# Indra-jith/failure-aware-vision

Measured on AMD Instinct MI355X. Metric: frames/sec, ResNet-50 MC-Dropout T=30 224x224 batch=256, higher is better.
Workload: dtype bf16; 1 GPU; BASELINE configs[2]: ResNet-50 v1.5 + MC-Dropout T=30 (all_blocks, p=0.10), 224x224x3 fp32 frames with Gaussian noise severity 3, batch 256 per GPU, synthetic frames and seeded synthetic weights; frames_per_gpu=256, global_batch=256, mc_samples=30, dropout_policy=all_blocks, inputs=resident in HBM before the timed region (H2D excluded), parallelism=batch sharded, 1 process per GPU, all-gather of (label, confidence)

## Files before the change

### failure_aware_vision_amd/csrc/fav.hip

```cpp
#include <hip/hip_runtime.h>

#include <algorithm>
#include <atomic>
#include <climits>
#include <cmath>
#include <cstdio>
#include <cstdlib>
#include <cstring>
#include <string>
#include <vector>

#include "../../include/fav.h"
#include "fav_kernels.hpp"
#include "fav_corrupt_c.hpp"
#include "fav_plan.hpp"
#include "fav_route.hpp"
#include "fav_views.hpp"
#include "fav_ood.hpp"
#include "fav_knn.hpp"

using namespace fav_plan;
using namespace fav_route;

namespace {
// ... 197 lines not shown
    igemm<128, 128, 64, 2, 0, 0>(), igemm<128, 128, 64, 2, 0, 1>(), igemm<128, 128, 64, 2, 0, 0, 0, true>(), igemm<128, 128, 64, 2, 0, 1, 0, true>(),
    igemm<128, 128, 64, 2, 1, 0>(), igemm<128, 128, 64, 2, 1, 1>(), igemm<128, 128, 64, 2, 1, 0, 0, true>(), igemm<128, 128, 64, 2, 1, 1, 0, true>(),
    igemm<256, 256, 64, 2, 0, 1, 1>(), igemm<256, 256, 64, 2, 0, 1, 1, true>(),
    igemm<256, 256, 64, 2, 0, 0>(), igemm<256, 256, 64, 2, 0, 1>(), igemm<256, 256, 64, 2, 0, 0, 0, true>(), igemm<256, 256, 64, 2, 0, 1, 0, true>(),
    igemm<256, 256, 64, 2, 1, 0>(), igemm<256, 256, 64, 2, 1, 1>(), igemm<256, 256, 64, 2, 1, 0, 0, true>(), igemm<256, 256, 64, 2, 1, 1, 0, true>(),
};
const KernelEntry<HaloKernel> kHaloKernels[] = {
    halo<64, 64, 256, 3, 1, 4, 0>(), halo<64, 64, 256, 3, 1, 4, 1>(), halo<128, 128, 256, 2, 2, 2, 0>(), halo<128, 128, 256, 2, 2, 2, 1>(),
    halo<64, 64, 128, 2, 1, 3, 0>(), halo<64, 64, 128, 2, 1, 3, 1>(), halo<128, 128, 128, 2, 1, 2, 0>(), halo<128, 128, 128, 2, 1, 2, 1>(),
};
const KernelEntry<TailKernel> kTailKernels[] = {
    tail<64, 0, true, 3, 4, true>(), tail<64, 0, true, 3, 4, false>(), tail<64, 64, true, 3, 4, true>(), tail<64, 64, true, 3, 4, false>(),
    tail<64, 128, true, 3, 4, true>(), tail<64, 128, true, 3, 4, false>(),
    tail<64, 0, false, 3, 4, true>(), tail<64, 0, false, 3, 4, false>(), tail<64, 64, false, 3, 4, true>(), tail<64, 64, false, 3, 4, false>(),
    tail<64, 128, false, 3, 4, true>(), tail<64, 128, false, 3, 4, false>(),
    tail<128, 0, true, 2, 8, true>(), tail<128, 0, true, 2, 8, false>(), tail<128, 128, true, 2, 8, true>(), tail<128, 128, true, 2, 8, false>(),
    tail<128, 0, false, 2, 8, true>(), tail<128, 0, false, 2, 8, false>(), tail<128, 128, false, 2, 8, true>(), tail<128, 128, false, 2, 8, false>(),
    tail<512, 0, false, 2, 8, true>(), tail<256, 0, true, 2, 8, true>(), tail<256, 0, false, 2, 4, true>(), tail<256, 0, false, 2, 4, false>(),
    tail<256, 256, false, 2, 8, true, 16>(), tail<256, 256, false, 2, 8, false, 16>(),
    tail<64, 64, true, 3, 4, true, 32, true>(), tail<64, 64, true, 3, 4, false, 32, true>(),
    {ROUTE_PROJ, {256, 512, 4}, bottleneck_tail_kernel<256, 0, false, 2, 4, true, 32, 512, false, false>},
    {ROUTE_PROJ, {512, 1024, 8}, bottleneck_tail_kernel<512, 0, false, 2, 8, true, 32, 1024, false, false>},
};
const KernelEntry<AttnKernel> kAttnKernels[] = {attn<0, 13, true>(), attn<0, 13>(), attn<0, 16>(), attn<1, 13>(), attn<1, 16>()};

template <class Fn, size_t N>
Fn find_kernel(const KernelEntry<Fn> (&table)[N], const Route& r, bool* lds_ok) {
    *lds_ok = true;
    for (const KernelEntry<Fn>& e : table) {
        if (e.kind != r.kind || memcmp(e.a, r.a, sizeof r.a) != 0) continue;
        if (r.lds > 0 && !e.lds_set.test_current()) {
            *lds_ok = hipFuncSetAttribute((const void*)e.fn, hipFuncAttributeMaxDynamicSharedMemorySize, 160 * 1024) == hipSuccess;
            if (*lds_ok) e.lds_set.set_current();
        }
        return e.fn;
    }
    return nullptr;
}

TailParams tail_params(const Route& r) {
    TailParams p;
    memset(&p, 0, sizeof p);
    p.H = r.Ho; p.W = r.Wo; p.HW = r.Ho * r.Wo; p.M = r.M;
    p.in_W = p.W; p.in_HW = p.HW; p.in_stride = 1;
    const TailGeom& g = r.geom;
    p.rega_bytes = g.rega_bytes;
    p.bias_b_off = g.bias_b_off; p.bias_ca_off = g.bias_ca_off; p.wa_off0 = g.wa_off0; p.wa_off1 = g.wa_off1; p.zero_off = g.zero_off;
    p.div_hw = fastdiv_make((uint32_t)p.HW);
    p.div_w = fastdiv_make((uint32_t)p.W);
    p.rs_T = r.rs_T; p.rs_tps = r.rs_tps;
    return p;
}

const char* launch_proj(fav_handle* h, const fav_conv_desc& d, const Route& r, const Group& G, hipStream_t s) {
    TailParams p = tail_params(r);
    p.t1 = (const uint16_t*)d.x; p.wc = (const uint16_t*)d.w; p.bias_c = d.bias; p.y = (uint16_t*)d.y;
    p.in_W = d.W; p.in_HW = d.H * d.W; p.in_stride = d.stride;
    p.drop = make_drop(nullptr);
    p.g_t1 = G.x; p.g_wc = G.w; p.g_bc = G.b; p.g_y = G.y;
    bool lds_ok;
    const TailKernel kern = find_kernel(kTailKernels, r, &lds_ok);
    if (!kern || !lds_ok) return kern ? "conv: cannot reserve LDS for the projection kernel" : "conv: no kernel for this route";
    const double flops = 2.0 * (double)r.M * d.Cin * d.Cout * G.n;
    const double bytes = 2.0 * ((double)r.M * (d.Cin + d.Cout) + (double)d.Cin * d.Cout) * G.n;
    Prof pr(h, s, FAV_K_CONV, flops, bytes);
    g_route = r;
    hipLaunchKernelGGL(kern, dim3(r.grid, r.groups), dim3(r.block), r.lds, s, p, 0);
    return nullptr;
}

const char* launch_conv(fav_handle* h, const fav_conv_desc& d, int cout_pad, int ldy, bool vit, const Group& G, hipStream_t s) {
    const Route r = route_conv(d, cout_pad, ldy, vit, G.n);
    if (r.refusal) return r.refusal;
    if (r.kind == ROUTE_PROJ) return launch_proj(h, d, r, G, s);
    ConvParams p;
    p.x = (const uint16_t*)d.x; p.w = (const uint16_t*)d.w; p.bias = d.bias; p.res = (const uint16_t*)d.res; p.y = d.y;
    p.H = d.H; p.W = d.W; p.Cin = d.Cin;
    p.Ho = r.Ho; p.Wo = r.Wo; p.HWo = r.Ho * r.Wo;
    p.Cout = d.Cout; p.ldy = ldy;
    p.kw = d.kw; p.stride = d.stride; p.pad = d.pad;
    p.M = r.M; p.K = r.K; p.nk = r.nk;
    p.relu = d.relu; p.out_f32 = d.out_f32;
    p.tiles_m = r.tiles_m; p.tiles_n = r.tiles_n; p.stage_mid = r.stage_mid;
    p.drop = make_drop(&d.drop);
    p.div_hwo = fastdiv_make((uint32_t)p.HWo);
    p.div_w = fastdiv_make((uint32_t)p.Wo);
    p.dbg = nullptr;
    p.g_x = G.x; p.g_w = G.w; p.g_bias = G.b; p.g_res = G.res; p.g_y = G.y;
    const bool halo = r.kind == ROUTE_CONV_HALO;
    bool lds_ok;
    const HaloKernel kern_halo = halo ? find_kernel(kHaloKernels, r, &lds_ok) : nullptr;
    const ConvKernel kern = halo ? nullptr : find_kernel(kConvKernels, r, &lds_ok);
    if (!kern_halo && !kern) return "conv: no kernel for this route";
    if (!lds_ok) return "conv: cannot reserve LDS for the staged 3x3 kernel";
    const double flops = 2.0 * (double)r.M * d.Cout * r.K * G.n;
    const double bytes = 2.0 * ((double)d.n_frames * d.H * d.W * d.Cin + (double)r.M * d.Cout * (d.res ? 2 : 1) * (d.out_f32 ? 2 : 1)
                                + (double)d.Cout * r.K) * G.n;
    const long long tiles = (long long)r.tiles_m * r.tiles_n;
    const bool dbg_on = FAV_KNOB("FAV_CONV_DBG", 0) != 0;
    if (dbg_on && !h) { (void)hipMalloc((void**)&p.dbg, (size_t)tiles * 32); (void)hipMemset(p.dbg, 0, (size_t)tiles * 32); }
    auto dbg_report = [&](long long nblocks, int bm, int bn, int bk) {
        if (!p.dbg) return;
        (void)hipStreamSynchronize(s);
        std::vector<unsigned long long> t((size_t)nblocks * 4);
        (void)hipMemcpy(t.data(), p.dbg, t.size() * 8, hipMemcpyDeviceToHost);
        (void)hipFree(p.dbg);
        unsigned long long lo = ~0ull, hi = 0;
        double ph[3] = {0, 0, 0};
        for (long long i = 0; i < nblocks; ++i) {
            lo = std::min(lo, t[i * 4]); hi = std::max(hi, t[i * 4 + 3]);
            for (int j = 0; j < 3; ++j) ph[j] += (double)(t[i * 4 + j + 1] - t[i * 4 + j]);
        }
        const double span = (double)(hi - lo), life = ph[0] + ph[1] + ph[2];
        fprintf(stderr, "[conv dbg] blocks %lld BMxBNxBK %dx%dx%d span %.1f us; per block: prologue %.2f us, k-loop %.2f us, epilogue %.2f us; "
                        "resident blocks/CU %.2f\n", nblocks, bm, bn, bk, span / 100.0, ph[0] / nblocks / 100.0, ph[1] / nblocks / 100.0,
                ph[2] / nblocks / 100.0, life / span / 256.0);
    };
    Prof pr(h, s, FAV_K_CONV, flops, bytes);
    g_route = r;
    if (halo) hipLaunchKernelGGL(kern_halo, dim3(r.grid, r.groups), dim3(r.block), r.lds, s, p, r.patch_bytes);
    else hipLaunchKernelGGL(kern, dim3(r.grid, r.groups), dim3(r.block), 0, s, p);
    dbg_report(r.grid, halo ? r.a[2] : r.a[0], r.a[1], halo ? 64 : r.a[2]);
    return nullptr;
}

const char* launch_tail(fav_handle* h, const fav_tail_desc& d, const Group& G, hipStream_t s) {
    const Route r = route_tail(d, G.n);
    if (r.refusal) return r.refusal;
    TailParams p = tail_params(r);
    p.t1 = (const uint16_t*)d.x; p.wb = (const uint16_t*)d.wb; p.bias_b = d.bias_b;
    p.wc = (const uint16_t*)d.wc; p.bias_c = d.bias_c; p.res = (const uint16_t*)d.res; p.y = (uint16_t*)d.y;
    p.wa = (const uint16_t*)d.wa; p.bias_a = d.bias_a; p.t1n = (uint16_t*)d.t1n;
    p.drop = make_drop(&d.drop);
    p.g_t1 = G.x; p.g_res = G.res; p.g_y = G.y; p.g_t1n = G.y2;
    p.g_wb = G.wb; p.g_bb = G.bb; p.g_wc = G.w; p.g_bc = G.b; p.g_wa = G.wa; p.g_ba = G.ba;
    p.site_e = d.entry_site;
    bool lds_ok;
    const TailKernel kern = find_kernel(kTailKernels, r, &lds_ok);
    if (!kern) return "bottleneck tail: unsupported shape";
    if (!lds_ok) return "bottleneck tail: cannot reserve LDS";
    const int cmid = d.Cmid, cout = 4 * cmid, nred = r.a[1], bm = r.geom.rp * r.geom.nw;
    const bool has3x3 = r.a[2] != 0;
    const long long M = r.M, nblocks = r.grid;
    const double flops = 2.0 * (double)M * ((has3x3 ? 9.0 * cmid * cmid : 0.0) + (double)cmid * cout + (double)cout * nred) * G.n;
    const double res_rows = d.res_entry ? (double)std::min<long long>(d.n_frames, p.drop.n_img) * p.HW : (double)M;
    const double bytes = 2.0 * ((double)M * (cmid + 1.0 * cout + nred) + res_rows * cout + (has3x3 ? 9.0 * cmid * cmid : 0.0) + (double)cmid * cout + (double)cout * nred) * G.n;
    Prof pr(h, s, FAV_K_CONV, flops, bytes);
    const bool dbg_on = FAV_KNOB("FAV_CONV_DBG", 0) != 0;
    if (dbg_on && !h) { (void)hipMalloc((void**)&p.dbg, (size_t)nblocks * 128); (void)hipMemset(p.dbg, 0, (size_t)nblocks * 128); }
    auto dbg_report = [&]() {
        if (!p.dbg) return;
        (void)hipStreamSynchronize(s);
        std::vector<unsigned long long> t((size_t)nblocks * 16);
        (void)hipMemcpy(t.data(), p.dbg, t.size() * 8, hipMemcpyDeviceToHost);
        (void)hipFree(p.dbg);
        if (const char* dump = fav_knob_str("FAV_CONV_DBG_DUMP")) {
            if (FILE* f = fopen(dump, "ab")) { const long long hdr[2] = {nblocks, cmid * 1000 + nred}; fwrite(hdr, 8, 2, f); fwrite(t.data(), 8, t.size(), f); fclose(f); }
        }
        unsigned long long lo = ~0ull, hi = 0;
        double ph[5] = {0, 0, 0, 0, 0};
        double cy[5] = {0, 0, 0, 0, 0};
        double cz[3] = {0, 0, 0};
        for (long long i = 0; i < nblocks; ++i) {
            lo = std::min(lo, t[i * 16]); hi = std::max(hi, t[i * 16 + 5]);
            unsigned long long prev = t[i * 16];
            for (int j = 0; j < 5; ++j) { const unsigned long long c = t[i * 16 + j + 1] ? t[i * 16 + j + 1] : prev; ph[j] += (double)(c - prev); prev = c; }
// ... 1907 lines not shown
```

### failure_aware_vision_amd/csrc/fav_kernels.hpp

```cpp
#pragma once
#include <hip/hip_runtime.h>
#include <float.h>
#include <stdint.h>

#ifdef FAV_EXPERIMENTS
#define FAV_DBG(P) ((P).dbg)
#else
#define FAV_DBG(P) ((unsigned long long*)nullptr)
#endif

namespace fav {

typedef __attribute__((__vector_size__(8 * sizeof(__bf16)))) __bf16 bf16x8_t;
typedef __attribute__((__vector_size__(4 * sizeof(float)))) float f32x4_t;

__device__ __forceinline__ float bf16_bits_to_f32(uint32_t b) { return __uint_as_float(b << 16); }

__device__ __forceinline__ uint32_t f32_to_bf16_bits(float f) {
    uint32_t u = __float_as_uint(f);
    return (u + 0x7FFFu + ((u >> 16) & 1u)) >> 16;
}
typedef __bf16 bf16x2_t __attribute__((ext_vector_type(2)));
typedef float f32x2_t __attribute__((ext_vector_type(2)));
typedef uint32_t u32x4_t __attribute__((ext_vector_type(4)));
// ... 328 lines not shown
            f32x4_t acc[4];
#pragma unroll
            for (int a = 0; a < 4; ++a) acc[a] = f32x4_t{0.f, 0.f, 0.f, 0.f};
#pragma unroll
            for (int s = 0; s < 6; ++s) {
                union { uint4 u; bf16x8_t v; } ub;
                ub.u = make_uint4(0, 0, 0, 0);
                if (s < 5) {
                    const StemFrag f = *(const StemFrag*)(win + 64 * s);
                    ub.u = s < 4 ? make_uint4(f.x, f.y, f.z, f.w) : make_uint4(f.x & km0, f.y & km1, f.z & km23, f.w & km23);
                }
#pragma unroll
                for (int a = 0; a < 4; ++a) {
                    union { uint4 u; bf16x8_t v; } ua;
                    ua.u = wf[a][s];
                    acc[a] = __builtin_amdgcn_mfma_f32_16x16x32_bf16(ua.v, ub.v, acc[a], 0, 0, 0);
                }
            }
            char* crow = (char*)conv_s + q * 128 + ((fq & 1) << 3);
#pragma unroll
            for (int a = 0; a < 4; ++a) {
                const float4 bq = *(const float4*)(bias_s + 16 * a + 4 * fq);
                const float v0 = __fadd_rn(acc[a][0], bq.x), v1 = __fadd_rn(acc[a][1], bq.y);
                const float v2 = __fadd_rn(acc[a][2], bq.z), v3 = __fadd_rn(acc[a][3], bq.w);
                *(uint2*)(crow + (((2 * a + (fq >> 1)) ^ (q & 7)) << 4)) = make_uint2(relu_bf16x2(pack_bf16x2(v0, v1)), relu_bf16x2(pack_bf16x2(v2, v3)));
            }
        }
        __syncthreads();

#pragma unroll
        for (int it = 0; it < 2; ++it) {
            const int item = tid + 256 * it;
            const int u = item & 7, pp = item >> 3;
            const int ppy = pp >> 3, ppx = pp & 7;
            const int gpy = py0 + ppy, gpx = px0 + ppx;
            if (gpy < p.Hp && gpx < p.Wp) {
                const int qm = (2 * ppy + 1) * CT + 2 * ppx + 1;
                u16x2_t best[4] = {{0, 0}, {0, 0}, {0, 0}, {0, 0}};
#pragma unroll
                for (int r = 0; r < 3; ++r) {
                    const bool rok = (unsigned)(2 * gpy - 1 + r) < (unsigned)p.Hc;
#pragma unroll
                    for (int s = 0; s < 3; ++s) {
                        const bool ok = rok && (unsigned)(2 * gpx - 1 + s) < (unsigned)p.Wc;
                        const int q = ok ? qm + (r - 1) * CT + (s - 1) : qm;
                        const uint4 v = *(const uint4*)((const char*)conv_s + q * 128 + ((u ^ (q & 7)) << 4));
                        best[0] = __builtin_elementwise_max(best[0], __builtin_bit_cast(u16x2_t, v.x));
                        best[1] = __builtin_elementwise_max(best[1], __builtin_bit_cast(u16x2_t, v.y));
                        best[2] = __builtin_elementwise_max(best[2], __builtin_bit_cast(u16x2_t, v.z));
                        best[3] = __builtin_elementwise_max(best[3], __builtin_bit_cast(u16x2_t, v.w));
                    }
                }
                *(uint4*)(p.out + (((img * p.Hp + gpy) * p.Wp + gpx) << 6) + 8 * u) =
                    make_uint4(__builtin_bit_cast(uint32_t, best[0]), __builtin_bit_cast(uint32_t, best[1]),
                               __builtin_bit_cast(uint32_t, best[2]), __builtin_bit_cast(uint32_t, best[3]));
            }
        }
    }
#undef FAV_STEM_REQUEST
}

__device__ __forceinline__ void lds_dma16(__amdgpu_buffer_rsrc_t srd, uint32_t voff, uint32_t soff, uint32_t lds_addr) {
    asm volatile("s_mov_b32 m0, %0\n\ts_nop 0\n\tbuffer_load_dwordx4 %1, %2, %3 offen lds"
                 :
                 : "s"(lds_addr), "v"(voff), "s"(srd), "s"(soff)
                 : "memory", "m0");
}

struct ConvParams {
    const uint16_t* x;
    const uint16_t* w;
    const float* bias;
    const uint16_t* res;
    void* y;
    int H, W, Cin, Ho, Wo, HWo;
    int Cout;
    int ldy;
    int kw, stride, pad;
    int M;
    int K, nk;
    int relu, out_f32;
    int tiles_m, tiles_n;
    int stage_mid;
    DropParams drop;
    FastDiv div_hwo;
    FastDiv div_w;
    unsigned long long* dbg;
    long long g_x, g_w, g_bias, g_res, g_y;
};

__device__ __forceinline__ ConvParams conv_group_params(const ConvParams& q) {
    ConvParams p = q;
    const long long g = blockIdx.y;
    p.x = (const uint16_t*)((const char*)q.x + g * q.g_x);
    p.w = (const uint16_t*)((const char*)q.w + g * q.g_w);
    p.bias = (const float*)((const char*)q.bias + g * q.g_bias);
    if (q.res) p.res = (const uint16_t*)((const char*)q.res + g * q.g_res);
    p.y = (void*)((char*)q.y + g * q.g_y);
    return p;
}

template <int BK>
__device__ __forceinline__ int lds_swz(int row) {
    return BK == 64 ? (row & 7) : ((-(row >> 2)) & 3);
}

constexpr int conv_waves_per_simd(int BM, int BN, int BK, int NS) {
    const int stage = NS * (BM + BN) * BK * 2, out = 64 * (BN + 4) * 4;
    const int lds = (stage > out ? stage : out) + BN * 5;
    int blocks = 163840 / lds;
    if (blocks > 4) blocks = 4;
    if (BN >= 128 && blocks > 3) blocks = 3;
    if (blocks < 1) blocks = 1;
    return blocks * (BM * 2 / 64) / 4;
}

template <int BM, int BN, int BK, int NS, int MODE, int WN = 2, int OCCW = 0, int EPI = 1, int PP = 0, bool GELU = false>
__global__ __launch_bounds__((BM / 64) * WN * 64, OCCW ? OCCW : conv_waves_per_simd(BM, BN, BK, NS)) void conv_igemm_kernel(const ConvParams p_launch) {
    const ConvParams p = conv_group_params(p_launch);
    constexpr int NT = (BM / 64) * WN * 64;
    constexpr int NWAVES = NT / 64;
    constexpr int ROWB = BK * 2;
    constexpr int CPR = BK / 8;
    constexpr int PROWS = 1024 / ROWB;
    constexpr int WTM = 64, WTN = BN / WN;
    constexpr int TM = WTM / 16, TN = WTN / 16;
    constexpr int A_BYTES = BM * ROWB, B_BYTES = BN * ROWB;
    constexpr int STAGE_BYTES = A_BYTES + B_BYTES;
    constexpr int OUT_LD = BN + 4;
    constexpr int OUT_BYTES = 64 * OUT_LD * 4;
    constexpr int LDS_BYTES = (EPI == 1 || NS * STAGE_BYTES > OUT_BYTES) ? NS * STAGE_BYTES : OUT_BYTES;
    constexpr int GS = WTN >= 64 ? 64 : 32;
    constexpr int CPL = GS / 4;
    constexpr int NG = WTN / GS;
    constexpr int AR = A_BYTES / 1024 / NWAVES, BR = B_BYTES / 1024 / NWAVES;
    __shared__ __attribute__((aligned(16))) unsigned char smem[LDS_BYTES + BN * 5];

    const int tid = threadIdx.x;
    const int lane = tid & 63;
    const int wave = tid >> 6;
    const int wm = wave / WN, wn = wave % WN;
    if (FAV_DBG(p) && tid == 0) FAV_DBG(p)[blockIdx.x * 4ull] = wall_clock64();

    const int nwg = gridDim.x;
    int tile;
    {
        const int b = blockIdx.x, xcd = b & 7, q = nwg >> 3, r = nwg & 7;
        tile = (xcd < r ? xcd * (q + 1) : r * (q + 1) + (xcd - r) * q) + (b >> 3);
    }
    const int tile_n = tile % p.tiles_n;
    const int tile_m = tile / p.tiles_n;
    const int m0 = tile_m * BM, n0 = tile_n * BN;
    if (tid < BN) ((float*)(smem + LDS_BYTES))[(tid >> 4) * 20 + (tid & 15)] = p.bias[n0 + tid];

    constexpr int NCH = BN / 16;
    constexpr int RPP = (NT / NCH > 64) ? 64 : NT / NCH;
    constexpr int NPASS = 64 / RPP;
    constexpr int NGROUPS = BM / 64;
    const int ec = tid % NCH, er = tid / NCH;
    const int n = n0 + ec * 16;
    const float* bias_s = (const float*)(smem + LDS_BYTES) + ec * 20;
    constexpr bool RES_ALL = NGROUPS * NPASS * 2 <= 8;
    constexpr int RG = RES_ALL ? NGROUPS : 1;
    u32x4_t rres[RG][NPASS][2];
    constexpr int RQ = CPL / 8;
    constexpr bool RES_ALL1 = TM * NG * RQ <= 8;
// ... 47 lines not shown
#pragma unroll
        for (int q_ = 0; q_ < NPASS; ++q_) rres[g_][q_][0] = rres[g_][q_][1] = (u32x4_t){0u, 0u, 0u, 0u};
    if (EPI == 0 && RES_ALL && p.res) {
#pragma unroll
        for (int g = 0; g < NGROUPS; ++g) FAV_LOAD_RES(g, g)
    }

    const int wave_u = __builtin_amdgcn_readfirstlane(wave);
    const int lrow = lane / CPR;
    const int lch = (lane % CPR) ^ lds_swz<BK>(lrow);
    const long long frame_elems = (long long)p.H * p.W * p.Cin;
    const int vimg0 = m0 / p.HWo;
    const int pad_shift = (p.pad * p.W + p.pad) * p.Cin;
    const __amdgpu_buffer_rsrc_t srd_a =
        __builtin_amdgcn_make_buffer_rsrc((void*)(p.x + vimg0 * frame_elems - pad_shift), 0, 0x7FFFFFFF, 0x00020000);
    const __amdgpu_buffer_rsrc_t srd_b =
        __builtin_amdgcn_make_buffer_rsrc((void*)(p.w + (long long)n0 * p.K), 0, BN * p.K * 2, 0x00020000);
    constexpr uint32_t OOB = 0x80000000u;
    uint32_t a_voff[AR];
    int a_ih0[AR], a_iw0[AR];
#pragma unroll
    for (int i = 0; i < AR; ++i) {
        const int m = m0 + (wave * AR + i) * PROWS + lrow;
        if (m < p.M) {
            const int vimg = (int)fastdiv((uint32_t)m, p.div_hwo);
            const int pix = m - vimg * p.HWo;
            const int oh = (int)fastdiv((uint32_t)pix, p.div_w), ow = pix - oh * p.Wo;
            a_ih0[i] = oh * p.stride - p.pad;
            a_iw0[i] = ow * p.stride - p.pad;
            a_voff[i] = (uint32_t)(((long long)(vimg - vimg0) * frame_elems +
                                    (long long)(a_ih0[i] * p.W + a_iw0[i]) * p.Cin + pad_shift + lch * 8) * 2);
        } else {
            a_ih0[i] = -0x40000000;
            a_iw0[i] = 0;
            a_voff[i] = OOB;
        }
    }
    uint32_t b_voff[BR];
#pragma unroll
    for (int i = 0; i < BR; ++i) {
        int r = (wave * BR + i) * PROWS + lrow;
        if (EPI == 1) r = (r & ~(GS - 1)) + CPL * ((r & 15) >> 2) + 4 * ((r >> 4) & (GS / 16 - 1)) + (r & 3);
        b_voff[i] = (uint32_t)((r * p.K + lch * 8) * 2);
    }
    const uint32_t lds_base =
        __builtin_amdgcn_readfirstlane((uint32_t)(uintptr_t)(const __attribute__((address_space(3))) void*)smem);
    const uint32_t lds_a = lds_base + wave_u * (AR * 1024);
    const uint32_t lds_b = lds_base + A_BYTES + wave_u * (BR * 1024);
    int tap_r = 0, tap_s = 0, c0 = 0;
    const bool has_taps = p.K != p.Cin || p.pad != 0 || p.stride != 1;

#define FAV_STAGE(BUF, KT)                                                                              \
    do {                                                                                                \
        const uint32_t soff_a = (uint32_t)(((tap_r * p.W + tap_s) * p.Cin + c0) * 2);                   \
        if (has_taps) {                                                                                 \
            _Pragma("unroll") for (int i = 0; i < AR; ++i) {                                            \
                const bool ok = (unsigned)(a_ih0[i] + tap_r) < (unsigned)p.H &&                         \
                                (unsigned)(a_iw0[i] + tap_s) < (unsigned)p.W;                           \
                lds_dma16(srd_a, ok ? a_voff[i] : OOB, soff_a, lds_a + (BUF) * STAGE_BYTES + i * 1024); \
            }                                                                                           \
        } else {                \
            _Pragma("unroll") for (int i = 0; i < AR; ++i)                                              \
                lds_dma16(srd_a, a_voff[i], soff_a, lds_a + (BUF) * STAGE_BYTES + i * 1024);            \
        }                                                                                               \
        _Pragma("unroll") for (int i = 0; i < BR; ++i)                                                  \
            lds_dma16(srd_b, b_voff[i], (uint32_t)((KT) * ROWB), lds_b + (BUF) * STAGE_BYTES + i * 1024); \
        c0 += BK;                                                                                       \
        if (c0 == p.Cin) {                                                                              \
            c0 = 0;                                                                                     \
            if (++tap_s == p.kw) { tap_s = 0; ++tap_r; }                                                \
        }                                                                                               \
    } while (0)

    f32x4_t acc[TN][TM];
#pragma unroll
    for (int a = 0; a < TN; ++a)
#pragma unroll
        for (int b = 0; b < TM; ++b) acc[a][b] = (f32x4_t){0.f, 0.f, 0.f, 0.f};

    const int frow = lane & 15;
    const int fq = lane >> 4;

    constexpr int PIECES = AR + BR;
#pragma unroll
    for (int t = 0; t < NS - 1; ++t)
        if (t < p.nk) FAV_STAGE(t, t);
    if (p.nk >= NS - 1) asm volatile("s_waitcnt vmcnt(%0)" ::"n"((NS - 2) * PIECES) : "memory");
    else asm volatile("s_waitcnt vmcnt(0)" ::: "memory");
    __syncthreads();
    if (FAV_DBG(p) && tid == 0) FAV_DBG(p)[blockIdx.x * 4ull + 1] = wall_clock64();

    int cur = 0, nxt = NS - 1;
    if constexpr (PP == 1) {
        static_assert(BK == 64 && NS == 2 && MODE == 0 && NT == 512, "ping-pong loop: 8 waves, 64-deep steps, two stages");
#define FAV_PP_READ(FX, FW, KK)                                                                          \
    do {                                                                                                \
        _Pragma("unroll") for (int b = 0; b < TM; ++b) {                                                \
            const int row = wm * WTM + b * 16 + frow;                                                   \
            FX[b] = *(const uint4*)(As + row * ROWB + ((((KK) * 4 + fq) ^ lds_swz<BK>(row)) << 4));     \
        }                                                                                               \
        _Pragma("unroll") for (int a = 0; a < TN; ++a) {                                                \
            const int row = wn * WTN + a * 16 + frow;                                                   \
            FW[a] = *(const uint4*)(Bs + row * ROWB + ((((KK) * 4 + fq) ^ lds_swz<BK>(row)) << 4));     \
        }                                                                                               \
    } while (0)
#define FAV_PP_MMA(FX, FW)                                                                               \
    do {                                                                                                \
        __builtin_amdgcn_s_setprio(1);                                                                  \
        _Pragma("unroll") for (int a = 0; a < TN; ++a)                                                  \
            _Pragma("unroll") for (int b = 0; b < TM; ++b) {                                            \
                union { uint4 u; bf16x8_t v; } ua, ub;                                                  \
                ua.u = FW[a]; ub.u = FX[b];                                                             \
                acc[a][b] = __builtin_amdgcn_mfma_f32_16x16x32_bf16(ua.v, ub.v, acc[a][b], 0, 0, 0);    \
            }                                                                                           \
        __builtin_amdgcn_s_setprio(0);                                                                  \
    } while (0)
#define FAV_PP_STEP_END()                                                                                \
    do {                                                                                                \
        asm volatile("s_waitcnt vmcnt(0)" ::: "memory");                                                \
        __syncthreads();                                                                                \
        cur ^= 1; nxt ^= 1;                                                                             \
    } while (0)
        if (wave_u < NWAVES / 2) {
            for (int kt = 0; kt < p.nk; ++kt) {
                const unsigned char* As = smem + cur * STAGE_BYTES;
                const unsigned char* Bs = As + A_BYTES;
                uint4 fx[TM], fw[TN];
                FAV_PP_READ(fx, fw, 0);
                if (kt + 1 < p.nk) FAV_STAGE(nxt, kt + 1);
                __builtin_amdgcn_sched_barrier(0);
                FAV_PP_MMA(fx, fw);
                __builtin_amdgcn_sched_barrier(0);
                FAV_PP_READ(fx, fw, 1);
                __builtin_amdgcn_sched_barrier(0);
                FAV_PP_MMA(fx, fw);
                __builtin_amdgcn_sched_barrier(0);
                FAV_PP_STEP_END();
            }
        } else {
            uint4 hx[TM], hw[TN];
            for (int kt = 0; kt < p.nk; ++kt) {
                const unsigned char* As = smem + cur * STAGE_BYTES;
                const unsigned char* Bs = As + A_BYTES;
                if (kt > 0) FAV_PP_MMA(hx, hw);
                if (kt + 1 < p.nk) FAV_STAGE(nxt, kt + 1);
                __builtin_amdgcn_sched_barrier(0);
                uint4 fx[TM], fw[TN];
                FAV_PP_READ(fx, fw, 0);
                __builtin_amdgcn_sched_barrier(0);
                FAV_PP_MMA(fx, fw);
                __builtin_amdgcn_sched_barrier(0);
                FAV_PP_READ(hx, hw, 1);
                asm volatile("s_waitcnt lgkmcnt(0)" ::: "memory");
                __builtin_amdgcn_sched_barrier(0);
                FAV_PP_STEP_END();
            }
            if (p.nk > 0) FAV_PP_MMA(hx, hw);
        }
#undef FAV_PP_READ
#undef FAV_PP_MMA
#undef FAV_PP_STEP_END
    } else
    for (int kt = 0; kt < p.nk; ++kt) {
        if ((BK == 32 || !p.stage_mid) && kt + NS - 1 < p.nk) FAV_STAGE(nxt, kt + NS - 1);
        const unsigned char* As = smem + cur * STAGE_BYTES;
        const unsigned char* Bs = As + A_BYTES;
#pragma unroll
        for (int kk = 0; kk < BK / 32; ++kk) {
            if (BK == 64 && kk == 1 && p.stage_mid && kt + NS - 1 < p.nk) FAV_STAGE(nxt, kt + NS - 1);
            uint4 fx[TM], fw[TN];
            const int ch = kk * 4 + fq;
#pragma unroll
            for (int b = 0; b < TM; ++b) {
                const int row = wm * WTM + b * 16 + frow;
                fx[b] = *(const uint4*)(As + row * ROWB + ((ch ^ lds_swz<BK>(row)) << 4));
            }
#pragma unroll
            for (int a = 0; a < TN; ++a) {
                const int row = wn * WTN + a * 16 + frow;
                fw[a] = *(const uint4*)(Bs + row * ROWB + ((ch ^ lds_swz<BK>(row)) << 4));
            }
            if (MODE == 0) {
#pragma unroll
                for (int a = 0; a < TN; ++a)
#pragma unroll
                    for (int b = 0; b < TM; ++b) {
                        union { uint4 u; bf16x8_t v; } ua, ub;
                        ua.u = fw[a];
                        ub.u = fx[b];
                        acc[a][b] = __builtin_amdgcn_mfma_f32_16x16x32_bf16(ua.v, ub.v, acc[a][b], 0, 0, 0);
                    }
            } else {
#pragma unroll
                for (int j = 0; j < 8; ++j) {
#pragma unroll
                    for (int a = 0; a < TN; ++a) {
                        const uint32_t wa = ((const uint32_t*)&fw[a])[j >> 1];
                        const float wf = bf16_bits_to_f32((j & 1) ? (wa >> 16) : (wa & 0xFFFFu));
#pragma unroll
                        for (int b = 0; b < TM; ++b) {
                            const uint32_t xa = ((const uint32_t*)&fx[b])[j >> 1];
                            const float xf = bf16_bits_to_f32((j & 1) ? (xa >> 16) : (xa & 0xFFFFu));
                            acc[a][b] = __builtin_amdgcn_mfma_f32_16x16x4f32(wf, xf, acc[a][b], 0, 0, 0);
                        }
                    }
                }
// ... 113 lines not shown
    for (int half = 0; half < NGROUPS; ++half) {
        const int rg = RES_ALL ? half : 0;
        if (!RES_ALL && p.res) FAV_LOAD_RES(0, half)
        if (half > 0) __syncthreads();
        if (wm == half) {
#pragma unroll
            for (int a = 0; a < TN; ++a)
#pragma unroll
                for (int b = 0; b < TM; ++b) {
                    const int ml = b * 16 + frow;
                    const int cw = (wn * WTN + a * 16) >> 4;
                    const int nl = cw * 16 + ((fq ^ (BN == 256 ? ((cw >> 3) & 1) * 2 : 0)) << 2);
                    *(f32x4_t*)(outs + ml * OUT_LD + nl) = acc[a][b];
                }
        }
        __syncthreads();
        if (!RES_ALL) FAV_RES_LANDED();
#pragma unroll
        for (int pass = 0; pass < NPASS; ++pass) {
            const int ml = er + pass * RPP;
            const int m = m0 + half * 64 + ml;
            if (er >= 64 || m >= p.M || n >= p.Cout) continue;
            uint32_t draws[4] = {~0u, ~0u, ~0u, ~0u};
            if (!p.out_f32 && p.drop.site >= 0) {
                const uint32_t vl = fastdiv((uint32_t)m, p.div_hwo);
                const uint32_t pix = (uint32_t)m - vl * (uint32_t)p.HWo;
                const uint32_t chunk = (uint32_t)(((long long)pix * p.Cout + n) >> 4);
                const uint4 w = drop_draws16(p.drop, (uint32_t)p.drop.v0 + vl, chunk);
                draws[0] = w.x; draws[1] = w.y; draws[2] = w.z; draws[3] = w.w;
            }
#pragma unroll
            for (int g = 0; g < 2; ++g) {
                float v[8];
#pragma unroll
                for (int q = 0; q < 2; ++q) {
                    const int gs = BN == 256 ? (g ^ ((ec >> 3) & 1)) : g;
                    const float4 t4 = *(const float4*)(outs + ml * OUT_LD + ec * 16 + 8 * gs + 4 * q);
                    const float4 bq = *(const float4*)(bias_s + 8 * g + 4 * q);
                    v[4 * q] = __fadd_rn(t4.x, bq.x); v[4 * q + 1] = __fadd_rn(t4.y, bq.y);
                    v[4 * q + 2] = __fadd_rn(t4.z, bq.z); v[4 * q + 3] = __fadd_rn(t4.w, bq.w);
                }
                if (p.res) {
                    const uint32_t rw[4] = {rres[rg][pass][g][0], rres[rg][pass][g][1], rres[rg][pass][g][2], rres[rg][pass][g][3]};
#pragma unroll
                    for (int j = 0; j < 4; ++j) {
                        v[2 * j] = __fadd_rn(v[2 * j], bf16_bits_to_f32(rw[j] & 0xFFFFu));
                        v[2 * j + 1] = __fadd_rn(v[2 * j + 1], bf16_bits_to_f32(rw[j] >> 16));
                    }
                }
                if (p.relu == 1) {
#pragma unroll
                    for (int j = 0; j < 8; ++j) v[j] = fmaxf(v[j], 0.f);
                } else if (GELU && p.relu == 2) {
#pragma unroll
                    for (int j = 0; j < 8; ++j) v[j] = fav_gelu(v[j]);
                }
                if (p.out_f32) {
                    float* yo = (float*)p.y + (long long)m * p.ldy + n + 8 * g;
#pragma unroll
                    for (int q = 0; q < 2; ++q)
                        if (n + 8 * g + 4 * q < p.Cout)
                            *(float4*)(yo + 4 * q) = make_float4(v[4 * q], v[4 * q + 1], v[4 * q + 2], v[4 * q + 3]);
                } else {
                    if (p.drop.site >= 0) {
#pragma unroll
                        for (int j = 0; j < 8; ++j)
                            v[j] = FAV_DROP_APPLY(v[j], draws, 8 * g + j, p.drop);
                    }
                    *(uint4*)((uint16_t*)p.y + (long long)m * p.ldy + n + 8 * g) =
                        make_uint4(pack_bf16x2(v[0], v[1]), pack_bf16x2(v[2], v[3]), pack_bf16x2(v[4], v[5]),
                                   pack_bf16x2(v[6], v[7]));
                }
            }
        }
    }
    }
    if (FAV_DBG(p)) {
        __syncthreads();
        if (tid == 0) FAV_DBG(p)[blockIdx.x * 4ull + 3] = wall_clock64();
    }
}

#undef FAV_STAGE
#undef FAV_LOAD_RES
#undef FAV_RES_LANDED
#undef FAV_LOAD_RES1
#undef FAV_RES1_LANDED

template <int CIN, int BN, int BM, int NS, int SUB, int OCC, int MODE>
__global__ __launch_bounds__(BM * 2, OCC) void conv3x3_halo_kernel(const ConvParams p_launch, int patch_bytes) {
    const ConvParams p = conv_group_params(p_launch);
    constexpr int NT = BM * 2, NWAVES = NT / 64;
    constexpr int ROWB = CIN * 2;
    constexpr int CPR = ROWB / 16;
    constexpr int PROWS = 1024 / ROWB;
    constexpr int CB = CIN / 64;
    constexpr int NKT = 9 * CB;
    constexpr int NSTEPS = NKT / SUB;
    constexpr bool RESIDENT = NS >= NSTEPS;
    constexpr int WAVES_M = BM / 64, WAVES_N = 2;
    constexpr int WTM = 64, WTN = BN / WAVES_N;
    constexpr int TM = WTM / 16, TN = WTN / 16;
    constexpr int B_BYTES = BN * 128;
    constexpr int BR = B_BYTES / 1024 / NWAVES;
    constexpr int OUT_LD = BN + 4;
    static_assert(NKT % SUB == 0 && BR >= 1 && WAVES_M * WAVES_N == NWAVES, "tile shape");
    extern __shared__ __attribute__((aligned(16))) unsigned char hsm[];
    unsigned char* const Bring = hsm + patch_bytes;
    float* const bias_s = (float*)(Bring + NS * SUB * B_BYTES);
    const uint32_t zero_off = ((uint32_t)(patch_bytes + NS * SUB * B_BYTES + BN * 5) + 255u) & ~255u;

    const int tid = threadIdx.x, lane = tid & 63, wave = tid >> 6;
    const int wm = wave / WAVES_N, wn = wave % WAVES_N;
    const int wave_u = __builtin_amdgcn_readfirstlane(wave);
    const int nwg = gridDim.x;
    int tile;
    {
        const int b = blockIdx.x, xcd = b & 7, q = nwg >> 3, r = nwg & 7;
        tile = (xcd < r ? xcd * (q + 1) : r * (q + 1) + (xcd - r) * q) + (b >> 3);
    }
    const int m0 = tile * BM;
    if (FAV_DBG(p) && tid == 0) FAV_DBG(p)[blockIdx.x * 4ull] = wall_clock64();
    if (tid < BN) bias_s[(tid >> 4) * 20 + (tid & 15)] = p.bias[tid];
    if (tid < 64) ((uint32_t*)(hsm + zero_off))[tid] = 0u;

    const uint32_t lds_base =
        __builtin_amdgcn_readfirstlane((uint32_t)(uintptr_t)(const __attribute__((address_space(3))) void*)hsm);
    const int W = p.W;
    const long long g0 = (long long)m0 - W - 1;
    const long long gbase = g0 > 0 ? g0 : 0;
    const __amdgpu_buffer_rsrc_t srd_a =
        __builtin_amdgcn_make_buffer_rsrc((void*)(p.x + gbase * CIN), 0, 0x7FFFFFFF, 0x00020000);
    constexpr uint32_t OOB = 0x80000000u;
    {
        const int npieces = patch_bytes >> 10;
        const int lrow = lane / CPR, lslot = lane % CPR;
        for (int j = wave_u; j < npieces; j += NWAVES) {
            const int q = j * PROWS + lrow;
            const int sw = (CPR == 8) ? (q & 7) : ((q & 7) | ((q & 1) << 3));
            const long long g = g0 + q;
            const bool ok = g >= 0 && g < (long long)p.M;
            const uint32_t voff = ok ? (uint32_t)((g - gbase) * ROWB + ((lslot ^ sw) << 4)) : OOB;
            lds_dma16(srd_a, voff, 0u, __builtin_amdgcn_readfirstlane(lds_base + (uint32_t)j * 1024u));
        }
    }
    const __amdgpu_buffer_rsrc_t srd_b =
        __builtin_amdgcn_make_buffer_rsrc((void*)p.w, 0, BN * p.K * 2, 0x00020000);
    uint32_t b_voff[BR];
    {
        const int lrow = lane >> 3, lch = (lane & 7) ^ (lrow & 7);
#pragma unroll
        for (int i = 0; i < BR; ++i) b_voff[i] = (uint32_t)((((wave * BR + i) * 8 + lrow) * p.K + lch * 8) * 2);
    }
    const uint32_t lds_b = lds_base + (uint32_t)patch_bytes + wave_u * (BR * 1024);
#define FAV_HSTAGE(BUF, STEP)                                                                          \
    do {                                                                                               \
        _Pragma("unroll") for (int u = 0; u < SUB; ++u)                                                \
            _Pragma("unroll") for (int i = 0; i < BR; ++i)                                             \
                lds_dma16(srd_b, b_voff[i], (uint32_t)(((STEP) * SUB + u) * 128),                      \
                          __builtin_amdgcn_readfirstlane(lds_b + ((BUF) * SUB + u) * B_BYTES + i * 1024)); \
    } while (0)
    constexpr int PIECES = BR * SUB;
    if (RESIDENT) {
#pragma unroll
        for (int t = 0; t < NSTEPS; ++t) FAV_HSTAGE(t, t);
    } else {
// ... 2310 lines not shown
```

### failure_aware_vision_amd/csrc/fav_route.hpp

```cpp
#pragma once

#include <cmath>
#include <cstdarg>
#include <cstdio>
#include <string>

#include "fav_plan.hpp"

namespace fav_route {

using namespace fav_plan;

enum RouteKind { ROUTE_NONE = 0, ROUTE_CONV_IGEMM, ROUTE_CONV_HALO, ROUTE_PROJ, ROUTE_TAIL, ROUTE_ATTENTION, ROUTE_ENTRY_REDUCE, ROUTE_STEM_POOL };

struct Route {
    int kind = ROUTE_NONE;
    int a[8] = {0, 0, 0, 0, 0, 0, 0, 0};
    bool fresh = true;
    const char* refusal = nullptr;
    unsigned grid = 0; int groups = 1;
    int block = 0, lds = 0;
    int patch_bytes = 0;
    int Ho = 0, Wo = 0, M = 0;
    int K = 0, nk = 0, tiles_m = 0, tiles_n = 0, stage_mid = 0;
    int rs_T = 0, rs_tps = 0;
    TailGeom geom = {};
};

inline Route refuse(const char* why) { Route r; r.refusal = why; return r; }

inline std::string fmt(const char* f, ...) {
    char buf[512];
    va_list ap;
    va_start(ap, f);
    vsnprintf(buf, sizeof buf, f, ap);
    va_end(ap);
    return buf;
}

inline std::string route_text(const Route& r) {
    const int* a = r.a;
    const char* mode = a[4] ? "f32" : "bf16";
    switch (r.kind) {
    case ROUTE_CONV_IGEMM:
        return fmt("conv_igemm<%d,%d,%d,%d,%s,epi%d%s%s>", a[0], a[1], a[2], a[3], mode, a[5], a[6] ? ",pp" : "", a[7] ? ",gelu" : "");
    case ROUTE_CONV_HALO:
        return fmt("conv3x3_halo<%d,%d,%d,%d,%s>", a[0], a[1], a[2], a[3], mode);
    case ROUTE_PROJ:
        return fmt("proj<%d,%d,nw%d>", a[0], a[1], a[2]);
    case ROUTE_TAIL:
        return fmt("tail<%d,%d,%s,nw%d,wc%d%s%s>", a[0], a[1], a[2] ? "3x3" : "1x1", a[3], a[4] ? 2 : 1, a[5] == 16 ? ",rp16" : "",
                   a[6] ? ",res_entry" : "");
    case ROUTE_ATTENTION:
        return fmt("attention<%s,%d%s>", a[0] ? "f32" : "bf16", a[1], a[2] ? ",full" : "");
    case ROUTE_ENTRY_REDUCE:
        return fmt("entry_reduce<%d,%d>", a[0], a[1]);
    case ROUTE_STEM_POOL:
        return fmt("stem7_pool<%s>", a[0] ? "f32" : "u8");
    default:
        return std::string();
    }
}

inline const char* check_drop(const char* who, const fav_dropout_desc* d, long long rows) {
    if (!d || d->site < 0) return nullptr;
    const char* why = nullptr;
    if (d->threshold > 255u) why = "dropout threshold above 255 (the draw is 8 bits wide: everything would be dropped)";
    else if (!std::isfinite(d->scale) || !(d->scale > 0.f)) why = "dropout scale must be finite and > 0";
    else if (d->n_img < 1) why = "dropout n_img must be >= 1";
    else if (d->v0 < 0 || d->v0 + rows > 0x7fffffffLL) why = "virtual frame index out of range";
    if (!why) return nullptr;
    thread_local std::string msg;
    msg = std::string(who) + ": " + why;
    return msg.c_str();
}

inline int conv_bk(int kh, int kw, int K, bool has_res) {
    const int forced = (int)FAV_KNOB("FAV_CONV_BK", 0);
    if (forced == 32 || forced == 64) return forced;
    return (kh * kw > 1 || (!has_res && K >= 512) || K >= 1024) ? 64 : 32;
}

inline bool conv_big(int kh, int kw, long long M, int cout_pad, int K, bool has_res) {
    const int mode = (int)FAV_KNOB("FAV_CONV_BIG", 2);
    const long long min_m = FAV_KNOB("FAV_CONV_BIG_MINM", 8192);
    if (mode == 0 || cout_pad % 256 != 0 || M < min_m) return false;
    if (mode == 1) return true;
    if ((M / 256) * (cout_pad / 256) < 512) return false;
    return kh * kw > 1 ? !has_res : K >= 512;
}

inline bool proj_enabled() { return FAV_KNOB("FAV_PROJ", 1) != 0; }

inline bool route_proj(const fav_conv_desc& d, int groups, Route* r) {
    const bool wide = d.Cin == 512 && d.Cout == 1024;
    if (!proj_enabled() || d.kh != 1 || d.kw != 1 || d.pad != 0 || !((d.Cin == 256 && d.Cout == 512) || wide) || d.res || d.drop.site >= 0 ||
        d.out_f32 || d.relu != 0 || d.math_mode != FAV_MATH_BF16 || (d.stride != 1 && d.stride != 2)) return false;
    const int Ho = conv_out(d.H, 1, d.stride, 0), Wo = conv_out(d.W, 1, d.stride, 0);
    const long long M = (long long)d.n_frames * Ho * Wo;
    if (M * groups < (wide ? 512 * 256 : 4096) || M > 0x7fffffffLL || (long long)d.H * d.W * d.Cin * 2 * 4 >= 0x40000000LL) return false;
    r->kind = ROUTE_PROJ;
    r->a[0] = d.Cin; r->a[1] = d.Cout; r->a[2] = wide ? 8 : 4;
    r->Ho = Ho; r->Wo = Wo; r->M = (int)M;
    TailGeom& g = r->geom;
    g.bias_b_off = 2 * 64 * d.Cin * 2; g.bias_ca_off = g.bias_b_off + d.Cin * 5; g.wa_off0 = g.wa_off1 = g.bias_b_off;
    g.zero_off = (g.bias_b_off + (d.Cin + d.Cout) * 5 + 255) & ~255;
    g.lds_bytes = g.zero_off + 256;
    g.nw = r->a[2]; g.rp = 32; g.wc2 = 1;
    r->grid = (unsigned)((M + 32 * g.nw - 1) / (32 * g.nw)); r->groups = groups;
    r->block = 64 * g.nw; r->lds = g.lds_bytes;
    return true;
}

inline Route route_conv(const fav_conv_desc& d, int cout_pad, int ldy, bool vit, int groups) {
    if (d.n_frames < 1 || d.H < 1 || d.W < 1) return refuse("conv: n_frames, H and W must be >= 1");
    if (d.kh < 1 || d.kw < 1 || d.stride < 1 || d.pad < 0) return refuse("conv: kh, kw and stride must be >= 1 and pad >= 0");
    if ((long long)d.H + 2ll * d.pad < d.kh || (long long)d.W + 2ll * d.pad < d.kw) return refuse("conv: the window does not fit the padded frame");
    if (d.relu < 0 || d.relu > 2) return refuse("conv: relu must be 0 (none), 1 (ReLU) or 2 (GELU)");
    if (d.out_f32 != 0 && d.out_f32 != 1) return refuse("conv: out_f32 must be 0 or 1");
    if (d.math_mode != FAV_MATH_BF16 && d.math_mode != FAV_MATH_F32_EXACT) return refuse("conv: unknown math_mode");
    if (d.Cin < 64 || d.Cin % 64 != 0) return refuse("conv: Cin must be a multiple of 64 and >= 64");
    if (d.Cout < 1 || cout_pad < d.Cout) return refuse("conv: Cout must be >= 1 and the padded Cout must cover it");
    if (cout_pad % 64 != 0) return refuse("conv: padded Cout must be a multiple of 64");
    if (!d.out_f32 && cout_pad != d.Cout) return refuse("conv: a bf16 output needs Cout to be a multiple of 64 (no column padding)");
    if (d.out_f32 && ldy < cout_pad) return refuse("conv: the fp32 output's row pitch must cover the padded Cout");
    Route r;
    if (cout_pad == d.Cout && ldy == d.Cout && route_proj(d, groups, &r)) return r;
    r.groups = groups;
    r.Ho = conv_out(d.H, d.kh, d.stride, d.pad);
    r.Wo = conv_out(d.W, d.kw, d.stride, d.pad);
    const int HWo = r.Ho * r.Wo;
    const long long M = (long long)d.n_frames * HWo;
    if (M <= 0 || M > 0x7fffffffLL) return refuse("conv: row count out of range");
    r.M = (int)M;
    r.K = d.kh * d.kw * d.Cin;
    if (const char* e = check_drop("conv", &d.drop, d.n_frames)) return refuse(e);
    if (d.out_f32 && d.drop.site >= 0) return refuse("conv: dropout on fp32 output unsupported");
    const int mode = d.math_mode == FAV_MATH_BF16 ? 0 : 1;
    const long long vit_big_tiles = FAV_KNOB("FAV_VIT_BIG_TILES", 50);
    const bool vit_big = vit && cout_pad % 256 == 0 && r.K >= 512 && (M / 256) * (cout_pad / 256) >= vit_big_tiles &&
                         FAV_KNOB("FAV_CONV_BIG", 2) != 0;
    const bool big = vit ? vit_big : conv_big(d.kh, d.kw, M * groups, cout_pad, r.K, d.res != nullptr);
    const int BN = big ? 256 : ((cout_pad % 128 == 0) ? 128 : 64);
    const int BK = big ? 64 : (vit ? 32 : conv_bk(d.kh, d.kw, r.K, d.res != nullptr));
    const int BM = big ? 256 : 128;
    r.stage_mid = (big && d.kh * d.kw > 1) ? 1 : 0;
    {
        const double frame_bytes = 2.0 * d.H * d.W * d.Cin;
        const double span = (BM / (double)HWo + 2.0) * frame_bytes + 2.0 * ((double)d.pad * d.W + d.pad) * d.Cin +
                            2.0 * (((double)d.kh * d.W + d.kw) * d.Cin);
        if (span >= 2147483647.0 || 2.0 * BN * (double)r.K >= 2147483647.0) return refuse("conv: frame too large for 32-bit tile offsets");
    }
    r.tiles_m = (r.M + BM - 1) / BM;
    r.tiles_n = cout_pad / BN;
    const long long tiles = (long long)r.tiles_m * r.tiles_n;
    if (tiles > 0x7fffffffLL) return refuse("conv: too many tiles");
    const int halo_mode = (int)FAV_KNOB("FAV_CONV_HALO", 1);
    if (halo_mode && d.kh == 3 && d.kw == 3 && d.stride == 1 && d.pad == 1 && !d.res && d.drop.site < 0 && !d.out_f32 &&
        (d.Cin == 64 || d.Cin == 128) && d.Cout == cout_pad && d.Cout == d.Cin && M * groups >= 2048) {
        const int halo_cfg = (int)FAV_KNOB("FAV_HALO_CFG", 1);
        const int HBM = halo_cfg == 0 ? 128 : 256;
        const int wstages = d.Cin == 64 ? (halo_cfg == 0 ? 2 : 3) : (halo_cfg == 0 ? 2 : 4);
        const int patch_bytes = (int)((((long long)(HBM + 2 * d.W + 2) * d.Cin * 2) + 1023) / 1024 * 1024);
        const int lds = patch_bytes + wstages * d.Cout * 128 + d.Cout * 5 + 512;
        if (lds <= 160 * 1024) {
            r.kind = ROUTE_CONV_HALO;
            r.a[0] = d.Cin; r.a[1] = d.Cout; r.a[2] = HBM; r.a[3] = (d.Cin == 64 && halo_cfg != 0) ? 3 : 2; r.a[4] = mode;
            r.nk = 9 * d.Cin / 64;
            r.grid = (unsigned)((r.M + HBM - 1) / HBM); r.block = HBM * 2; r.lds = lds; r.patch_bytes = patch_bytes;
            return r;
        }
    }
    r.nk = r.K / BK;
    const int epi_forced = (int)FAV_KNOB("FAV_CONV_EPI", -1);
    const int epi = epi_forced >= 0 ? epi_forced : ((d.res && !big) ? 0 : 1);
    const int pp = (big && epi && (int)FAV_KNOB("FAV_CONV_PP", 1) && mode == 0) ? 1 : 0;
    r.kind = ROUTE_CONV_IGEMM;
    r.a[0] = BM; r.a[1] = BN; r.a[2] = BK; r.a[3] = BK == 32 ? 3 : 2; r.a[4] = mode; r.a[5] = epi ? 1 : 0; r.a[6] = pp; r.a[7] = d.relu == 2;
    r.grid = (unsigned)tiles; r.block = BM * 2;
    return r;
}

inline Route route_tail(const fav_tail_desc& d, int groups) {
    if (d.n_frames < 1 || d.H < 1 || d.W < 1) return refuse("bottleneck tail: n_frames, H and W must be >= 1");
    const bool has3x3 = d.wb != nullptr;
    const int nred = d.wa ? d.Nred : 0;
    Route r;
    TailGeom& g = r.geom;
    if (!tail_geometry(d.Cmid, nred, has3x3, d.W, &g)) return refuse("bottleneck tail: unsupported shape");
    const int HW = d.H * d.W;
    const long long M = (long long)d.n_frames * d.H * d.W;
    if (M <= 0 || M > 0x7fffffffLL) return refuse("bottleneck tail: row count out of range");
    if (const char* e = check_drop("bottleneck tail", &d.drop, d.n_frames)) return refuse(e);
    if (d.res_entry) {
        if (!(d.Cmid == 64 && nred == 64 && has3x3) || d.drop.site < 0 || d.entry_site < 0 || !d.res)
            return refuse("bottleneck tail: res_entry needs Cmid = Nred = 64 with the 3x3 and both dropout sites");
        if ((double)d.drop.n_img * HW * 4.0 * d.Cmid * 2.0 >= 2147483647.0) return refuse("bottleneck tail: cached tensor too large for 32-bit offsets");
    }
    { const int lds_pad = (int)FAV_KNOB("FAV_TAIL_LDS_PAD", 0); if (g.lds_bytes + lds_pad <= 160 * 1024) g.lds_bytes += lds_pad; }
    const int bm = g.rp * g.nw;
    if (d.res_entry) {
        const bool sample_minor = FAV_KNOB("FAV_ENTRY_RES_ORDER", 1) != 0;
        const long long sample_rows = (long long)d.drop.n_img * HW;
        if (sample_minor && d.drop.v0 % d.drop.n_img == 0 && d.n_frames % d.drop.n_img == 0 && sample_rows % bm == 0) {
            r.rs_T = d.n_frames / d.drop.n_img;
            r.rs_tps = (int)(sample_rows / bm);
        }
    }
    r.kind = ROUTE_TAIL;
    r.a[0] = d.Cmid; r.a[1] = nred; r.a[2] = has3x3; r.a[3] = g.nw; r.a[4] = g.wc2; r.a[5] = g.rp; r.a[6] = d.res_entry != 0;
    r.Ho = d.H; r.Wo = d.W; r.M = (int)M;
    r.grid = (unsigned)((M + bm - 1) / bm); r.groups = groups;
    r.block = g.nw * 64; r.lds = g.lds_bytes; r.patch_bytes = g.patch_bytes;
    return r;
}

inline Route route_attention(int n, int T, int D, int heads, int math_mode) {
    if (T < 1 || T > 256 || heads * 64 != D || n < 1) return refuse("attention: need 1 <= tokens <= 256 and 64-wide heads");
    const int nkt = (T + 15) / 16, Tp2 = (T + 31) / 32 * 32;
    const int rounds = (nkt + 7) / 8;
    int nw = (nkt + rounds - 1) / rounds;
    const int attn_nw = (int)FAV_KNOB("FAV_ATTN_WAVES", 0);
    if (attn_nw >= 1 && attn_nw <= 8) nw = attn_nw;
    Route r;
    r.kind = ROUTE_ATTENTION;
    r.a[0] = math_mode == FAV_MATH_BF16 ? 0 : 1; r.a[1] = nkt <= 13 ? 13 : 16; r.a[2] = r.a[0] == 0 && nkt == 13;
    r.M = T;
    r.grid = (unsigned)(n * heads); r.block = nw * 64; r.lds = nkt * 16 * 128 + Tp2 * 128;
    return r;
}

}
```

Before: 3500 frames/s.

## Add eight-phase interleaved K loop for ping-pong conv GEMM on 1x1 convs

Adds an alternative main loop for the ping-pong implicit-GEMM conv kernel. It splits each K step into four sub-phases, with LDS fragment reads, global-to-LDS DMA staging of the next tiles, and MFMA bursts interleaved and separated by barriers. The aim is finer-grained overlap of memory traffic with matrix math in the big 1x1 convolutions. The router enables it by default for 1x1 convs and ViT shapes, and an env knob can override it. It adds more barriers per K step and more register pressure from the extra fragment buffers.

```diff
diff --git a/failure_aware_vision_amd/csrc/fav.hip b/failure_aware_vision_amd/csrc/fav.hip
--- a/failure_aware_vision_amd/csrc/fav.hip
+++ b/failure_aware_vision_amd/csrc/fav.hip
@@ -303,6 +303,7 @@
     p.M = r.M; p.K = r.K; p.nk = r.nk;
     p.relu = d.relu; p.out_f32 = d.out_f32;
     p.tiles_m = r.tiles_m; p.tiles_n = r.tiles_n; p.stage_mid = r.stage_mid;
+    p.kloop = r.kloop;
     p.drop = make_drop(&d.drop);
     p.div_hwo = fastdiv_make((uint32_t)p.HWo);
     p.div_w = fastdiv_make((uint32_t)p.Wo);
diff --git a/failure_aware_vision_amd/csrc/fav_kernels.hpp b/failure_aware_vision_amd/csrc/fav_kernels.hpp
--- a/failure_aware_vision_amd/csrc/fav_kernels.hpp
+++ b/failure_aware_vision_amd/csrc/fav_kernels.hpp
@@ -434,6 +434,7 @@
     int relu, out_f32;
     int tiles_m, tiles_n;
     int stage_mid;
+    int kloop;
     DropParams drop;
     FastDiv div_hwo;
     FastDiv div_w;
@@ -647,11 +648,53 @@
     const int fq = lane >> 4;
 
     constexpr int PIECES = AR + BR;
-#pragma unroll
-    for (int t = 0; t < NS - 1; ++t)
-        if (t < p.nk) FAV_STAGE(t, t);
-    if (p.nk >= NS - 1) asm volatile("s_waitcnt vmcnt(%0)" ::"n"((NS - 2) * PIECES) : "memory");
-    else asm volatile("s_waitcnt vmcnt(0)" ::: "memory");
+#define FAV_K8_STAGE_PX(BUF, HU)                                                                        \
+    do {                                                                                                \
+        const uint32_t soff_a = (uint32_t)(((tap_r * p.W + tap_s) * p.Cin + c0) * 2);                   \
+        if (has_taps) {                                                                                 \
+            _Pragma("unroll") for (int i = 2 * (HU); i < 2 * (HU) + 2; ++i) {                           \
+                const bool ok = (unsigned)(a_ih0[i] + tap_r) < (unsigned)p.H &&                         \
+                                (unsigned)(a_iw0[i] + tap_s) < (unsigned)p.W;                           \
+                lds_dma16(srd_a, ok ? a_voff[i] : OOB, soff_a, lds_a + (BUF) * STAGE_BYTES + i * 1024); \
+            }                                                                                           \
+        } else {                                                                                        \
+            _Pragma("unroll") for (int i = 2 * (HU); i < 2 * (HU) + 2; ++i)                             \
+                lds_dma16(srd_a, a_voff[i], soff_a, lds_a + (BUF) * STAGE_BYTES + i * 1024);            \
+        }                                                                                               \
+        if ((HU) == 1) {                                                                                \
+            c0 += BK;                                                                                   \
+            if (c0 == p.Cin) {                                                                          \
+                c0 = 0;                                                                                 \
+                if (++tap_s == p.kw) { tap_s = 0; ++tap_r; }                                            \
+            }                                                                                           \
+        }                                                                                               \
+    } while (0)
+#define FAV_K8_STAGE_W(BUF, GU, KT)                                                                     \
+    do {                                                                                                \
+        _Pragma("unroll") for (int i = 2 * (GU); i < 2 * (GU) + 2; ++i)                                 \
+            lds_dma16(srd_b, b_voff[i], (uint32_t)((KT) * ROWB), lds_b + (BUF) * STAGE_BYTES + i * 1024); \
+    } while (0)
+    bool k8 = false;
+    if constexpr (PP == 1) k8 = p.kloop != 0;
+    if (k8) {
+        if constexpr (PP == 1) {
+            static_assert(AR == 4 && BR == 4, "eight-phase loop: two pieces per wave and unit");
+            FAV_K8_STAGE_PX(0, 0); FAV_K8_STAGE_PX(0, 1);
+            FAV_K8_STAGE_W(0, 0, 0); FAV_K8_STAGE_W(0, 1, 0);
+            if (p.nk > 1) {
+                FAV_K8_STAGE_PX(1, 0); FAV_K8_STAGE_PX(1, 1);
+                asm volatile("s_waitcnt vmcnt(4)" ::: "memory");
+            } else {
+                asm volatile("s_waitcnt vmcnt(0)" ::: "memory");
+            }
+        }
+    } else {
+#pragma unroll
+        for (int t = 0; t < NS - 1; ++t)
+            if (t < p.nk) FAV_STAGE(t, t);
+        if (p.nk >= NS - 1) asm volatile("s_waitcnt vmcnt(%0)" ::"n"((NS - 2) * PIECES) : "memory");
+        else asm volatile("s_waitcnt vmcnt(0)" ::: "memory");
+    }
     __syncthreads();
     if (FAV_DBG(p) && tid == 0) FAV_DBG(p)[blockIdx.x * 4ull + 1] = wall_clock64();
 
@@ -686,7 +729,81 @@
         __syncthreads();                                                                                \
         cur ^= 1; nxt ^= 1;                                                                             \
     } while (0)
-        if (wave_u < NWAVES / 2) {
+        if (k8) {
+            static_assert(TM == 4 && TN == 8, "eight-phase loop: 64 x 128 wave tile");
+#define FAV_K8_BAR()                                            \
+    do {                                                        \
+        __builtin_amdgcn_sched_barrier(0);                      \
+        __builtin_amdgcn_s_barrier();                           \
+        asm volatile("" ::: "memory");                          \
+        __builtin_amdgcn_sched_barrier(0);                      \
+    } while (0)
+#define FAV_K8_READ_PX(FX, PH)                                                                           \
+    do {                                                                                                \
+        _Pragma("unroll") for (int kk = 0; kk < 2; ++kk)                                                \
+            _Pragma("unroll") for (int b = 0; b < 2; ++b) {                                             \
+                const int row = wm * WTM + ((PH) * 2 + b) * 16 + frow;                                  \
+                FX[kk][b] = *(const uint4*)(As + row * ROWB + (((kk * 4 + fq) ^ lds_swz<BK>(row)) << 4)); \
+            }                                                                                           \
+    } while (0)
+#define FAV_K8_READ_W(CH)                                                                                \
+    do {                                                                                                \
+        _Pragma("unroll") for (int kk = 0; kk < 2; ++kk)                                                \
+            _Pragma("unroll") for (int a = 0; a < 4; ++a) {                                             \
+                const int row = wn * WTN + ((CH) * 4 + a) * 16 + frow;                                  \
+                fw8[kk][a] = *(const uint4*)(Bs + row * ROWB + (((kk * 4 + fq) ^ lds_swz<BK>(row)) << 4)); \
+            }                                                                                           \
+    } while (0)
+#define FAV_K8_MMA(FX, PH, CH)                                                                           \
+    do {                                                                                                \
+        __builtin_amdgcn_s_setprio(1);                                                                  \
+        _Pragma("unroll") for (int kk = 0; kk < 2; ++kk)                                                \
+            _Pragma("unroll") for (int a = 0; a < 4; ++a)                                               \
+                _Pragma("unroll") for (int b = 0; b < 2; ++b) {                                         \
+                    union { uint4 u; bf16x8_t v; } ua, ub;                                              \
+                    ua.u = fw8[kk][a]; ub.u = FX[kk][b];                                                \
+                    acc[(CH) * 4 + a][(PH) * 2 + b] =                                                   \
+                        __builtin_amdgcn_mfma_f32_16x16x32_bf16(ua.v, ub.v, acc[(CH) * 4 + a][(PH) * 2 + b], 0, 0, 0); \
+                }                                                                                       \
+        __builtin_amdgcn_s_setprio(0);                                                                  \
+    } while (0)
+            const bool late = wave_u >= NWAVES / 2;
+            if (late) FAV_K8_BAR();
+            uint4 fx0[2][2], fx1[2][2], fw8[2][4];
+            for (int kt = 0; kt < p.nk; ++kt) {
+                const unsigned char* As = smem + cur * STAGE_BYTES;
+                const unsigned char* Bs = As + A_BYTES;
+                FAV_K8_READ_PX(fx0, 0);
+                FAV_K8_READ_W(0);
+                if (kt + 1 < p.nk) FAV_K8_STAGE_W(nxt, 0, kt + 1);
+                FAV_K8_BAR();
+                FAV_K8_MMA(fx0, 0, 0);
+                FAV_K8_BAR();
+                FAV_K8_READ_PX(fx1, 1);
+                if (kt + 1 < p.nk) FAV_K8_STAGE_W(nxt, 1, kt + 1);
+                asm volatile("s_waitcnt lgkmcnt(0)" ::: "memory");
+                FAV_K8_BAR();
+                FAV_K8_MMA(fx1, 1, 0);
+                FAV_K8_BAR();
+                FAV_K8_READ_W(1);
+                if (kt + 2 < p.nk) FAV_K8_STAGE_PX(cur, 0);
+                asm volatile("s_waitcnt lgkmcnt(0)" ::: "memory");
+                FAV_K8_BAR();
+                FAV_K8_MMA(fx1, 1, 1);
+                FAV_K8_BAR();
+                if (kt + 2 < p.nk) { FAV_K8_STAGE_PX(cur, 1); asm volatile("s_waitcnt vmcnt(4)" ::: "memory"); }
+                else asm volatile("s_waitcnt vmcnt(0)" ::: "memory");
+                FAV_K8_BAR();
+                FAV_K8_MMA(fx0, 0, 1);
+                FAV_K8_BAR();
+                cur ^= 1; nxt ^= 1;
+            }
+            if (!late) FAV_K8_BAR();
+#undef FAV_K8_BAR
+#undef FAV_K8_READ_PX
+#undef FAV_K8_READ_W
+#undef FAV_K8_MMA
+        } else if (wave_u < NWAVES / 2) {
             for (int kt = 0; kt < p.nk; ++kt) {
                 const unsigned char* As = smem + cur * STAGE_BYTES;
                 const unsigned char* Bs = As + A_BYTES;
@@ -966,6 +1083,8 @@
 }
 
 #undef FAV_STAGE
+#undef FAV_K8_STAGE_PX
+#undef FAV_K8_STAGE_W
 #undef FAV_LOAD_RES
 #undef FAV_RES_LANDED
 #undef FAV_LOAD_RES1
diff --git a/failure_aware_vision_amd/csrc/fav_route.hpp b/failure_aware_vision_amd/csrc/fav_route.hpp
--- a/failure_aware_vision_amd/csrc/fav_route.hpp
+++ b/failure_aware_vision_amd/csrc/fav_route.hpp
@@ -22,7 +22,7 @@
     int block = 0, lds = 0;
     int patch_bytes = 0;
     int Ho = 0, Wo = 0, M = 0;
-    int K = 0, nk = 0, tiles_m = 0, tiles_n = 0, stage_mid = 0;
+    int K = 0, nk = 0, tiles_m = 0, tiles_n = 0, stage_mid = 0, kloop = 0;
     int rs_T = 0, rs_tps = 0;
     TailGeom geom = {};
 };
@@ -175,6 +175,15 @@
     const int epi_forced = (int)FAV_KNOB("FAV_CONV_EPI", -1);
     const int epi = epi_forced >= 0 ? epi_forced : ((d.res && !big) ? 0 : 1);
     const int pp = (big && epi && (int)FAV_KNOB("FAV_CONV_PP", 1) && mode == 0) ? 1 : 0;
+    if (pp) {
+        const bool one = d.kh * d.kw == 1;
+        int k8 = 0;
+        if (!vit && one) k8 = 1;
+        if (!vit && !one && d.stride == 2) k8 = 0;
+        if (vit) k8 = 1;
+        const int forced = (int)FAV_KNOB("FAV_CONV_KLOOP", -1);
+        r.kloop = forced >= 0 ? (forced != 0) : k8;
+    }
     r.kind = ROUTE_CONV_IGEMM;
     r.a[0] = BM; r.a[1] = BN; r.a[2] = BK; r.a[3] = BK == 32 ? 3 : 2; r.a[4] = mode; r.a[5] = epi ? 1 : 0; r.a[6] = pp; r.a[7] = d.relu == 2;
     r.grid = (unsigned)tiles; r.block = BM * 2;
```

Result: no change. 3523 frames/s (median of 6 runs) (+0.6%).
